# Dustin-Ray/capyCRYPT

Measured on NVIDIA B200. Metric: sha3_256_GBps, higher is better.
Workload: dtype u64

## Files before the change

### capycrypt_b200/csrc/sha3_api.cu

```cuda
#include <algorithm>
#include <cmath>
#include <cstdlib>
#include <memory>
#include <thread>
#include <type_traits>
#include <vector>

#include "internal.h"
#include "hostbatch.h"
#include "sponge.cuh"

namespace capy {

template <int LANES>
__global__ void __launch_bounds__(128)
    sha3_uniform_kernel(const uint8_t* __restrict__ data, uint64_t stride, uint64_t len, uint32_t suffix,
                        uint8_t* __restrict__ out, uint32_t out_bytes, uint64_t n) {
  const uint64_t i = (uint64_t)blockIdx.x * blockDim.x + threadIdx.x;
  if (i >= n) return;
  constexpr uint64_t RATE = 8ull * LANES;
  const uint2* q = reinterpret_cast<const uint2*>(data + i * stride);
  Lane a[25];
  state_zero(a);
  const uint64_t nfull = len / RATE;
  for (uint64_t b = 0; b < nfull; b++) {
#pragma unroll
    for (int j = 0; j < LANES; j++) {
      uint2 v = __ldg(q + j);
      a[j].lo ^= v.x;
      a[j].hi ^= v.y;
    }
    q += LANES;
    keccak_f1600(a);
  }
  const uint32_t rem = (uint32_t)(len - nfull * RATE);
#pragma unroll
  for (int j = 0; j < LANES; j++) {
    const uint32_t o = 8u * j;
    uint32_t lo = 0, hi = 0;
    if (o < rem) {
      uint2 v = __ldg(q + j);
      lo = v.x;
      hi = v.y;
      if (o + 8 > rem) {
        const uint32_t keep = rem - o;
        if (keep < 4) {
          lo &= (1u << (8 * keep)) - 1u;
          hi = 0;
        } else if (keep > 4) {
          hi &= (1u << (8 * (keep - 4))) - 1u;
        } else {
          hi = 0;
        }
      }
    }
    if (rem >= o && rem < o + 8) {
      const uint32_t k = rem - o;
      if (k < 4) lo |= suffix << (8 * k);
      else hi |= suffix << (8 * (k - 4));
    }
    a[j].lo ^= lo;
    a[j].hi ^= hi;
  }
  if (rem + 1 < RATE) a[LANES - 1].hi ^= 0x80000000u;
  keccak_f1600(a);

  uint8_t* o = out + i * (uint64_t)out_bytes;
  if ((out_bytes & 15u) == 0 && (reinterpret_cast<uintptr_t>(out) & 15u) == 0) {
#pragma unroll
    for (int j = 0; j < 4; j++)
      if (16u * j < out_bytes)
        reinterpret_cast<uint4*>(o)[j] = make_uint4(a[2 * j].lo, a[2 * j].hi, a[2 * j + 1].lo, a[2 * j + 1].hi);
  } else {
#pragma unroll
    for (int j = 0; j < 8; j++) {
      if (8u * j < out_bytes) reinterpret_cast<uint32_t*>(o)[2 * j] = a[j].lo;
      if (8u * j + 4 < out_bytes) reinterpret_cast<uint32_t*>(o)[2 * j + 1] = a[j].hi;
    }
  }
}

template <int LANES, int MSG_LANES>
__global__ void __launch_bounds__(128)
    sha3_short_kernel(const uint4* __restrict__ data, uint64_t stride16, uint32_t suffix, uint4* __restrict__ out,
                      uint32_t out_bytes, uint64_t n) {
  static_assert(MSG_LANES % 2 == 0 && MSG_LANES < LANES, "whole 16-byte loads, one block");
  const uint64_t i = (uint64_t)blockIdx.x * blockDim.x + threadIdx.x;
  if (i >= n) return;
  const uint4* q = data + i * stride16;
  Lane a[25];
  state_zero(a);
#pragma unroll
  for (int j = 0; j < MSG_LANES / 2; j++) {
    const uint4 v = __ldg(q + j);
    a[2 * j].lo = v.x;
    a[2 * j].hi = v.y;
    a[2 * j + 1].lo = v.z;
    a[2 * j + 1].hi = v.w;
  }
  a[MSG_LANES].lo = suffix;
  a[LANES - 1].hi ^= 0x80000000u;
  keccak_round(a, KECCAK_RC[0]);
#pragma unroll 1
  for (int r = 1; r < 23; r += 2) {
    keccak_round(a, KECCAK_RC[r]);
    keccak_round(a, KECCAK_RC[r + 1]);
  }
  keccak_round(a, KECCAK_RC[23]);
  uint4* o = out + i * (uint64_t)(out_bytes / 16);
#pragma unroll
  for (int j = 0; j < 4; j++)
    if (16u * j < out_bytes) o[j] = make_uint4(a[2 * j].lo, a[2 * j].hi, a[2 * j + 1].lo, a[2 * j + 1].hi);
}

template <int LANES>
__global__ void prefix_state_kernel(const uint8_t* prefix, uint32_t nblocks, uint64_t* state) {
  if (threadIdx.x != 0 || blockIdx.x != 0) return;
  Lane a[25];
  state_zero(a);
  for (uint32_t b = 0; b < nblocks; b++) {
    const uint8_t* p = prefix + (size_t)b * 8 * LANES;
#pragma unroll
    for (int j = 0; j < LANES; j++) {
      uint64_t v = 0;
      for (int k = 0; k < 8; k++) v |= (uint64_t)p[8 * j + k] << (8 * k);
      a[j].lo ^= (uint32_t)v;
      a[j].hi ^= (uint32_t)(v >> 32);
    }
    keccak_f1600(a);
  }
  for (int k = 0; k < 25; k++) state[k] = ((uint64_t)a[k].hi << 32) | a[k].lo;
}

constexpr uint32_t kLenBins = 1u << 14;
constexpr uint64_t kHostPlanMaxItems = 1ull << 18;

__device__ __forceinline__ uint32_t len_bin(const uint64_t* off, uint64_t i, uint32_t stride_bytes) {
  const uint64_t blocks = (off[i + 1] - off[i]) / stride_bytes;
  return blocks < kLenBins - 1 ? (uint32_t)blocks : kLenBins - 1;
}

__global__ void len_hist_kernel(const uint64_t* __restrict__ off, uint64_t n, uint32_t stride_bytes, uint32_t* hist) {
  const uint64_t i = (uint64_t)blockIdx.x * blockDim.x + threadIdx.x;
  if (i < n) atomicAdd(&hist[len_bin(off, i, stride_bytes)], 1u);
}

__global__ void __launch_bounds__(1024) len_scan_kernel(uint32_t* hist, uint32_t* summary) {
  __shared__ unsigned long long tot_s;
  __shared__ uint32_t max_s, bins_s;
  const uint32_t t = threadIdx.x;
  constexpr uint32_t PER = kLenBins / 1024;
  static_assert(PER == 16, "four uint4 per thread");
  if (t == 0) { tot_s = 0; max_s = 0; bins_s = 0; }
  __syncthreads();
  const uint32_t lo = kLenBins - (t + 1) * PER;
  uint32_t c[PER];
#pragma unroll
  for (int q = 0; q < 4; q++) {
    const uint4 v = reinterpret_cast<const uint4*>(hist + lo)[q];
    c[4 * q] = v.x; c[4 * q + 1] = v.y; c[4 * q + 2] = v.z; c[4 * q + 3] = v.w;
  }
  uint32_t sum = 0, nb = 0, mx = 0;
  unsigned long long tot = 0;
#pragma unroll
  for (int k = 0; k < (int)PER; k++) {
    sum += c[k];
    if (c[k]) { nb++; mx = lo + k; }
    tot += (unsigned long long)c[k] * (lo + k + 1);
  }
  if (sum) {
    atomicAdd(&tot_s, tot);
    atomicMax(&max_s, mx);
    atomicAdd(&bins_s, nb);
  }
  __syncthreads();
  uint32_t incl = sum;
#pragma unroll
  for (int d = 1; d < 32; d <<= 1) {
    const uint32_t v = __shfl_up_sync(0xffffffffu, incl, d);
    if ((t & 31) >= (uint32_t)d) incl += v;
  }
  __shared__ uint32_t wsum[32];
  if ((t & 31) == 31) wsum[t >> 5] = incl;
  __syncthreads();
  if (t < 32) {
    uint32_t w = wsum[t];
#pragma unroll
    for (int d = 1; d < 32; d <<= 1) {
      const uint32_t v = __shfl_up_sync(0xffffffffu, w, d);
      if (t >= (uint32_t)d) w += v;
    }
    wsum[t] = w;
  }
  __syncthreads();
  uint32_t run = incl - sum + ((t >> 5) ? wsum[(t >> 5) - 1] : 0u);
#pragma unroll
  for (int k = (int)PER - 1; k >= 0; k--) {
    const uint32_t cnt = c[k];
    c[k] = run;
    run += cnt;
  }
#pragma unroll
  for (int q = 0; q < 4; q++) reinterpret_cast<uint4*>(hist + lo)[q] = make_uint4(c[4 * q], c[4 * q + 1], c[4 * q + 2], c[4 * q + 3]);
  if (t == 0) {
    summary[0] = (uint32_t)tot_s;
    summary[1] = (uint32_t)(tot_s >> 32);
    summary[2] = max_s;
    summary[3] = bins_s;
  }
}

__global__ void len_scatter_kernel(const uint64_t* __restrict__ off, uint64_t n, uint32_t stride_bytes, uint32_t* cursor,
                                   uint32_t* __restrict__ order) {
  const uint64_t i = (uint64_t)blockIdx.x * blockDim.x + threadIdx.x;
  if (i < n) order[atomicAdd(&cursor[len_bin(off, i, stride_bytes)], 1u)] = (uint32_t)i;
}

constexpr double kPairChainRatio = 3.08 / 4.6;
constexpr int kMaxWarpCosched = 3;
constexpr double kWarpChainRatio[kMaxWarpCosched + 1] = {0.0, 2.06 / 4.6, 2.36 / 4.6, 3.00 / 4.6};

static void plan_tiers(const std::vector<uint32_t>& cum, uint64_t n, uint32_t max_blocks, double total_blocks, int sm_count,
                       uint64_t warp_items[kMaxWarpCosched], uint64_t* pair_items, int force_c = 0) {
  for (int c = 0; c < kMaxWarpCosched; c++) warp_items[c] = 0;
  *pair_items = 0;
  const size_t nb = cum.size();
  std::vector<double> work_above(nb);
  double acc = 0;
  for (size_t k = nb; k-- > 0;) {
    work_above[k] = acc;
    const uint64_t cnt = (k == 0 ? n : cum[k - 1]) - cum[k];
    acc += (double)cnt * (double)(k + 1);
  }
  auto longer_than = [&](double thr, uint64_t* count, double* work) {
    if (thr < 1.0) {
      *count = n;
      *work = total_blocks;
      return;
    }
    const size_t k = std::min<size_t>((size_t)thr - 1, nb - 1);
    *count = cum[k];
    *work = work_above[k];
  };
  const double l1 = (double)max_blocks;
  const int c_first = force_c >= 1 && force_c <= kMaxWarpCosched ? force_c : 1;
  for (double T = l1 * kWarpChainRatio[c_first]; T < l1; T *= 1.01) {
    uint64_t k_above[kMaxWarpCosched + 2];
    double w_above[kMaxWarpCosched + 2];
    k_above[0] = 0;
    w_above[0] = 0;
    for (int c = 1; c <= kMaxWarpCosched; c++) {
      const int next = c + 1;
      const double ratio = next <= kMaxWarpCosched ? kWarpChainRatio[next] : kPairChainRatio;
      longer_than(T / ratio, &k_above[c], &w_above[c]);
      if (force_c && c != force_c) {
        k_above[c] = c < force_c ? 0 : k_above[force_c];
        w_above[c] = c < force_c ? 0 : w_above[force_c];
      }
    }
    uint64_t k_fast;
    double w_fast;
    longer_than(T, &k_fast, &w_fast);
    if (k_above[kMaxWarpCosched] == 0 && T < l1 * kPairChainRatio) continue;
    uint64_t blocks = 0;
    double sm_time = 0;
    uint64_t cnt[kMaxWarpCosched];
    for (int c = 1; c <= kMaxWarpCosched; c++) {
      cnt[c - 1] = k_above[c] - k_above[c - 1];
      blocks += (cnt[c - 1] + 4 * c - 1) / (4 * c);
      sm_time += (w_above[c] - w_above[c - 1]) * kWarpChainRatio[c] / (4.0 * c);
    }
    const uint64_t k_p = k_fast - k_above[kMaxWarpCosched];
    blocks += (k_p + 63) / 64;
    sm_time += (w_fast - w_above[kMaxWarpCosched]) * kPairChainRatio / 64.0 + (total_blocks - w_fast) / 128.0;
    if (blocks + 1 > (uint64_t)sm_count) continue;
    if (sm_time > 0.95 * T * (double)sm_count) continue;
    if ((total_blocks - w_fast) / 128.0 > T * (double)((uint64_t)sm_count - blocks)) continue;
    for (int c = 0; c < kMaxWarpCosched; c++) warp_items[c] = cnt[c];
    *pair_items = k_p;
    return;
  }
}

template <int... Ls, class F>
static int with_lanes(int lanes, F&& f) {
  int rc = CAPY_ERR_BAD_ARG;
  (void)((lanes == Ls && ((rc = f(std::integral_constant<int, Ls>())), true)) || ...);
  return rc;
}

struct CudaFree {
  void operator()(void* p) const { cudaFree(p); }
};
template <class T>
using DevPtr = std::unique_ptr<T, CudaFree>;
template <class T>
static cudaError_t dev_alloc(DevPtr<T>& p, size_t bytes) {
  T* q = nullptr;
  const cudaError_t e = cudaMalloc(&q, bytes);
  if (e == cudaSuccess) p.reset(q);
  return e;
}

struct LenHist {
  uint64_t total_blocks = 0;
  uint32_t max_bin = 0;
  uint32_t bins = 0;
  std::vector<uint32_t> cnt;
};

static void host_len_hist(const uint64_t* h_off, uint64_t n, uint32_t stride_bytes, LenHist* h) {
  h->cnt.assign(kLenBins, 0);
  const double inv = 1.0 / (double)stride_bytes;
  for (uint64_t i = 0; i < n; i++) {
    const uint64_t len = h_off[i + 1] - h_off[i];
    uint64_t q = (uint64_t)((double)len * inv);
    if (q * stride_bytes > len) q--;
    else if ((q + 1) * stride_bytes <= len) q++;
    const uint32_t b = q < kLenBins - 1 ? (uint32_t)q : kLenBins - 1;
    if (h->cnt[b]++ == 0) h->bins++;
    if (b > h->max_bin) h->max_bin = b;
    h->total_blocks += (uint64_t)b + 1;
  }
}

static int device_len_hist(capy_ctx* ctx, cudaStream_t st, const uint64_t* d_off, uint64_t n, uint32_t stride_bytes,
                           uint32_t* hist, LenHist* h) {
  uint32_t* summary = hist + kLenBins;
  CAPY_CUDA(ctx, cudaMemsetAsync(hist, 0, (size_t)kLenBins * 4 + 64, st));
  len_hist_kernel<<<(unsigned)((n + 255) / 256), 256, 0, st>>>(d_off, n, stride_bytes, hist);
  len_scan_kernel<<<1, 1024, 0, st>>>(hist, summary);
  ctx->launches += 2;
  if (!h->cnt.empty()) return CAPY_OK;
  uint32_t h_sum[4];
  CAPY_CUDA(ctx, cudaMemcpyAsync(h_sum, summary, sizeof h_sum, cudaMemcpyDeviceToHost, st));
  CAPY_CUDA(ctx, cudaStreamSynchronize(st));
  h->total_blocks = (uint64_t)h_sum[0] | ((uint64_t)h_sum[1] << 32);
  h->max_bin = h_sum[2];
  h->bins = h_sum[3];
  return CAPY_OK;
}

static int plan_from_hist(capy_ctx* ctx, DeviceCtx& dc, cudaStream_t st, const uint64_t* d_off, uint64_t n,
                          uint32_t stride_bytes, const LenHist& h, uint32_t* hist, uint32_t* order, bool allow_pair,
                          int force_c, LaunchPlan* plan) {
  const uint32_t max_blocks = h.max_bin + 1;
  const double ideal = (double)h.total_blocks / (32.0 * 4.0 * dc.sm_count);
  if (allow_pair && max_blocks > 64 && (double)max_blocks > 1.05 * ideal) {
    std::vector<uint32_t> cum(kLenBins);
    if (!h.cnt.empty()) {
      uint32_t above = 0;
      for (uint32_t k = kLenBins; k-- > 0;) {
        cum[k] = above;
        above += h.cnt[k];
      }
    } else {
      CAPY_CUDA(ctx, cudaMemcpyAsync(cum.data(), hist, (size_t)kLenBins * 4, cudaMemcpyDeviceToHost, st));
      CAPY_CUDA(ctx, cudaStreamSynchronize(st));
    }
    plan_tiers(cum, n, max_blocks, (double)h.total_blocks, dc.sm_count, plan->warp_items, &plan->pair_items, force_c);
  }
  if (h.bins == 1) plan->uniform_blocks = max_blocks;
  if (h.bins > 1) {
    len_scatter_kernel<<<(unsigned)((n + 255) / 256), 256, 0, st>>>(d_off, n, stride_bytes, hist, order);
    ctx->launches++;
    CAPY_CUDA(ctx, cudaGetLastError());
    plan->order = order;
    plan->warps_per_smsp = 0;
    if ((double)max_blocks * 4.0 > 0.7 * ideal) {
      plan->warps_per_smsp = 3;
      if ((double)max_blocks * 3.0 > 0.7 * ideal) plan->warps_per_smsp = 2;
      if ((double)max_blocks * 2.0 > 0.7 * ideal) plan->warps_per_smsp = 1;
    }
  }
  return CAPY_OK;
}

static int plan_ragged(capy_ctx* ctx, DeviceCtx& dc, cudaStream_t st, const uint64_t* d_off, uint64_t n,
                       uint32_t stride_bytes, LaunchPlan* plan, bool allow_pair = true, int force_c = 0) {
  *plan = LaunchPlan();
  if (n < 1 || n > 0xffffffffull) return CAPY_OK;
  const uint64_t* h_off = host_off_find(dc, d_off, n);
  LenHist h;
  if (h_off) {
    const uint64_t len0 = h_off[1] - h_off[0];
    bool uniform = true;
    for (uint64_t i = 1; i < n && uniform; i++) uniform = (h_off[i + 1] - h_off[i]) == len0;
    if (uniform) {
      plan->uniform_blocks = len0 / stride_bytes + 1;
      return CAPY_OK;
    }
    if (n > kHostPlanMaxItems) h_off = nullptr;
    else host_len_hist(h_off, n, stride_bytes, &h);
  }
  const bool cached = ctx->plan_cache.load() != 0 && force_c == 0 && !h_off;
  if (cached) {
    for (PlanEntry& e : dc.plans)
      if (e.off == d_off && e.n == n && e.unit == stride_bytes && e.allow_pair == allow_pair) {
        e.last_use = ++dc.use_clock;
        *plan = e.plan;
        return CAPY_OK;
      }
  }
  uint32_t* hist = (uint32_t*)scratch_get(dc, st, kPlanHist, (size_t)kLenBins * 4 + 64);
  DevPtr<uint32_t> owned;
  if (cached && dev_alloc(owned, (size_t)n * 4) != cudaSuccess) {
    cudaGetLastError();
    return CAPY_ERR_OOM;
  }
  uint32_t* order = cached ? owned.get() : (uint32_t*)scratch_get(dc, st, kPlanOrder, (size_t)n * 4);
  if (!hist || !order) return CAPY_ERR_OOM;
  int rc = device_len_hist(ctx, st, d_off, n, stride_bytes, hist, &h);
  if (rc) return rc;
  rc = plan_from_hist(ctx, dc, st, d_off, n, stride_bytes, h, hist, order, allow_pair, force_c, plan);
  if (rc) return rc;
  if (cached) {
    if (!plan->order) owned.reset();
    if (dc.plans.size() >= kMaxPlanEntries) {
      size_t lru = 0;
      for (size_t k = 1; k < dc.plans.size(); k++)
        if (dc.plans[k].last_use < dc.plans[lru].last_use) lru = k;
      if (dc.plans[lru].owned_order) cudaFree(dc.plans[lru].owned_order);
      dc.plans.erase(dc.plans.begin() + lru);
    }
    PlanEntry e;
    e.off = d_off;
    e.n = n;
    e.unit = stride_bytes;
    e.allow_pair = allow_pair;
    e.plan = *plan;
    e.owned_order = owned.release();
    e.last_use = ++dc.use_clock;
    dc.plans.push_back(e);
  }
  return CAPY_OK;
}

template <class Kernel>
static cudaError_t throttle(Kernel* kernel, const LaunchPlan& plan, unsigned* block, size_t* smem) {
  *smem = 0;
  if (plan.warps_per_smsp < 1 || plan.warps_per_smsp > 3) return cudaSuccess;
  *block = 128;
  *smem = (size_t)(227 * 1024 / plan.warps_per_smsp) - 1024;
  return cudaFuncSetAttribute(kernel, cudaFuncAttributeMaxDynamicSharedMemorySize, 226 * 1024);
}

template <int LANES>
static int launch_sponge_t(capy_ctx* ctx, cudaStream_t stream, SpongeJob J, unsigned block, const LaunchPlan& plan) {
  if (plan.tiered()) {
    const uint64_t warp_items = plan.warp_items[0] + plan.warp_items[1] + plan.warp_items[2], pair_items = plan.pair_items;
    SpongeTiers tiers;
    uint32_t warp_blocks = 0;
    uint64_t rank = 0;
    for (int c = 0; c < 3; c++) {
      tiers.first_block[c] = warp_blocks;
      tiers.first_rank[c] = rank;
      warp_blocks += grid_for(plan.warp_items[c], 4 * (c + 1));
      rank += plan.warp_items[c];
    }
    tiers.warp_blocks = warp_blocks;
    tiers.pair_blocks = grid_for(2 * pair_items, 128);
    const unsigned solo_blocks = grid_for(J.n - pair_items - warp_items, 128);
    J.warp_items = warp_items;
    J.first = warp_items + pair_items;
    CAPY_CUDA(ctx, cudaFuncSetAttribute(sponge_tiered_kernel<LANES>, cudaFuncAttributeMaxDynamicSharedMemorySize, 226 * 1024));
    sponge_tiered_kernel<LANES><<<warp_blocks + tiers.pair_blocks + solo_blocks, 384, 226 * 1024, stream>>>(J, tiers);
    ctx->launches++;
    CAPY_CUDA(ctx, cudaGetLastError());
    return CAPY_OK;
  }
  size_t smem;
  CAPY_CUDA(ctx, throttle(sponge_kernel<LANES>, plan, &block, &smem));
  sponge_kernel<LANES><<<grid_for(J.n, block), block, smem, stream>>>(J);
  ctx->launches++;
  CAPY_CUDA(ctx, cudaGetLastError());
  return CAPY_OK;
}

static unsigned pick_block(uint64_t n, int sm_count, int threads_per_sm) {
  unsigned best = 128;
  double best_eff = -1.0;
  for (unsigned bs : {128u, 64u, 32u}) {
    const uint64_t blocks = (n + bs - 1) / bs;
    const uint64_t slots = (uint64_t)sm_count * (threads_per_sm / bs);
    const uint64_t waves = (blocks + slots - 1) / slots;
    const double per_sm = (double)blocks / sm_count;
    const double busiest = waves > 1 ? (double)waves * (threads_per_sm / bs) : (double)((blocks + sm_count - 1) / sm_count);
    const double eff = per_sm / busiest;
    if (eff > best_eff + 0.02) {
      best_eff = eff;
      best = bs;
    }
  }
  return best;
}

static int job_lanes(const SpongeJob& J) { return (int)(J.rate / 8); }

static int launch_sponge(capy_ctx* ctx, DeviceCtx& dc, cudaStream_t stream, const SpongeJob& J, const LaunchPlan& plan) {
  if (J.n == 0) return CAPY_OK;
  const unsigned block = pick_block(J.n, dc.sm_count, 384);
  return with_lanes<9, 13, 17, 18, 19, 21>(job_lanes(J), [&](auto L) {
    return launch_sponge_t<decltype(L)::value>(ctx, stream, J, block, plan);
  });
}

static int launch_sponge_seq(capy_ctx* ctx, DeviceCtx& dc, cudaStream_t stream, const SpongeJob& A, const SpongeJob& B,
                             const LaunchPlan& plan) {
  const int rc = launch_sponge(ctx, dc, stream, A, plan);
  if (rc) return rc;
  return launch_sponge(ctx, dc, stream, B, plan);
}

static bool chain_jobs_fit(int sm_count, uint64_t n) {
  if (getenv("CAPY_NO_CHAIN_SPLIT") || sm_count < 1) return false;
  return (n + 127) / 128 >= (uint64_t)CAPY_SPONGE_MINB * (uint64_t)sm_count;
}

static bool chain_cut(int sm_count, uint64_t n, uint64_t absorb_blocks, uint64_t squeeze_extra, uint64_t* cut) {
  if (!chain_jobs_fit(sm_count, n)) return false;
  const uint64_t warps = (n + 31) / 32, sched = 4ull * (uint64_t)sm_count;
  if (warps > 8 * sched) return false;
  auto fill = [&](uint64_t w) {
    const double x = (double)w / (double)sched;
    return x / std::ceil(x);
  };
  if (fill(2 * warps) < fill(warps) + 0.04) return false;
  const uint64_t perms = absorb_blocks + squeeze_extra;
  if (perms < 12) return false;
  uint64_t k = (perms + 1) / 2;
  if (k > absorb_blocks) k = absorb_blocks;
  if (3 * k < perms) return false;
  *cut = k;
  return true;
}

static int launch_chain_jobs(capy_ctx* ctx, DeviceCtx& dc, cudaStream_t stream, const SpongeJob& J0, const SpongeJob& J1,
                             bool data_dependent) {
  const uint32_t nb = (uint32_t)((J0.n + 127) / 128);
  uint32_t* sync = (uint32_t*)scratch_get(dc, stream, kChainSync, ((size_t)nb + 1) * sizeof(uint32_t));
  if (!sync) return CAPY_ERR_OOM;
  CAPY_CUDA(ctx, cudaMemsetAsync(sync, 0, ((size_t)nb + 1) * sizeof(uint32_t), stream));
  SpongeChain C;
  C.j[0] = J0;
  C.j[1] = J1;
  C.sync = sync;
  C.blocks_per_job = nb;
  C.data_dependent = data_dependent ? 1u : 0u;
  return with_lanes<9, 13, 17, 18, 19, 21>(job_lanes(J0), [&](auto L) {
    sponge_chain_kernel<decltype(L)::value><<<2 * nb, 128, 0, stream>>>(C);
    ctx->launches++;
    CAPY_CUDA(ctx, cudaGetLastError());
    return CAPY_OK;
  });
}

static int launch_sponge_chain(capy_ctx* ctx, DeviceCtx& dc, cudaStream_t stream, const SpongeJob& J, uint64_t cut) {
  uint64_t* states = (uint64_t*)scratch_get(dc, stream, kChainStates, (size_t)J.n * 25 * sizeof(uint64_t));
  if (!states) return CAPY_ERR_OOM;
  SpongeJob J0 = J, J1 = J;
  J0.chain_out = states;
  J0.stop_block = J.skip_blocks + cut;
  J1.chain_in = states;
  J1.skip_blocks = (uint32_t)(J.skip_blocks + cut);
  return launch_chain_jobs(ctx, dc, stream, J0, J1, false);
}

static bool uniform_cut(const DeviceCtx& dc, const SpongeJob& J, const LaunchPlan& plan, uint64_t* cut) {
  if (J.out_off || J.xor_in || plan.order || (J.rate & 7u) != 0) return false;
  const uint64_t msg_blocks = J.off ? plan.uniform_blocks : J.msg_len / J.rate + 1;
  if (!msg_blocks) return false;
  uint64_t absorb = msg_blocks;
  if (J.keys) absorb += ((uint64_t)J.key_len + 8) / J.w + 1;
  if (!J.skip_blocks) absorb += J.prefix_len / J.rate;
  const uint64_t sq = 8ull * J.sq_lanes, squeeze_extra = J.out_bytes ? (J.out_bytes + sq - 1) / sq - 1 : 0;
  return chain_cut(dc.sm_count, J.n, absorb, squeeze_extra, cut);
}

static int run_sponge(capy_ctx* ctx, DeviceCtx& dc, cudaStream_t stream, SpongeJob J, const LaunchPlan& plan) {
  J.order = plan.order;
  uint64_t cut;
  if (uniform_cut(dc, J, plan, &cut)) return launch_sponge_chain(ctx, dc, stream, J, cut);
  return launch_sponge(ctx, dc, stream, J, plan);
}

static int launch_sha3(capy_ctx* ctx, DeviceCtx& dc, cudaStream_t stream, int d, const uint8_t* data, const uint64_t* off,
                       uint64_t msg_len, uint64_t stride, uint64_t n, uint8_t* out, uint32_t flags = 0,
                       bool tail_readable = true) {
  if (!valid_secparam(d)) return CAPY_ERR_BAD_SECPARAM;
  if (n == 0) return CAPY_OK;
  if (!off && !tail_readable && (msg_len & 7u) != 0 && n > 1 && (reinterpret_cast<uintptr_t>(data) & 7u) == 0 &&
      (stride & 7u) == 0 && (reinterpret_cast<uintptr_t>(out) & 3u) == 0) {
    int rc = launch_sha3(ctx, dc, stream, d, data, nullptr, msg_len, stride, n - 1, out, flags, true);
    if (rc) return rc;
    return launch_sha3(ctx, dc, stream, d, data + (n - 1) * stride, nullptr, msg_len, stride, 1, out + (n - 1) * (uint64_t)(d / 8),
                       flags, false);
  }
  const uint32_t rate = (1600 - sha3_capacity(d)) / 8;
  const int lanes = (int)rate / 8;
  if (!off && (reinterpret_cast<uintptr_t>(data) & 15u) == 0 && (reinterpret_cast<uintptr_t>(out) & 15u) == 0 &&
      (stride & 15u) == 0 && (d == 256 || d == 512) && msg_len >= 16 && (msg_len & 15u) == 0 && msg_len < rate) {
    const unsigned block = 128, grid = grid_for(n, block);
    const uint4* dq = reinterpret_cast<const uint4*>(data);
    uint4* oq = reinterpret_cast<uint4*>(out);
    const uint64_t s16 = stride / 16;
    const int msg_lanes = (int)(msg_len / 8);
    const int rc = d == 256 ? with_lanes<2, 4, 6, 8, 10, 12, 14, 16>(msg_lanes, [&](auto M) {
      sha3_short_kernel<17, decltype(M)::value><<<grid, block, 0, stream>>>(dq, s16, 0x06u, oq, 32, n);
      return CAPY_OK;
    }) : with_lanes<2, 4, 6, 8>(msg_lanes, [&](auto M) {
      sha3_short_kernel<9, decltype(M)::value><<<grid, block, 0, stream>>>(dq, s16, 0x06u, oq, 64, n);
      return CAPY_OK;
    });
    if (rc) return rc;
    ctx->launches++;
    CAPY_CUDA(ctx, cudaGetLastError());
    return CAPY_OK;
  }
  SpongeJob J{};
  J.data = data;
  J.off = off;
  J.msg_len = msg_len;
  J.msg_stride = stride;
  J.trailer_len = 1;
  J.sha3_suffix = 1;
  J.rate = rate;
  J.out = out;
  J.out_stride = J.out_bytes = (uint64_t)d / 8;
  J.sq_lanes = (1600 - d) / 64;
  J.n = n;
  uint64_t cut;
  if (!off && !uniform_cut(dc, J, LaunchPlan(), &cut) && (reinterpret_cast<uintptr_t>(data) & 7u) == 0 &&
      (stride & 7u) == 0 && (reinterpret_cast<uintptr_t>(out) & 3u) == 0 && (tail_readable || (msg_len & 7u) == 0)) {
    const uint32_t suffix = (msg_len % 136u == 135u) ? 0x86u : 0x06u;
    const unsigned block = 128, grid = grid_for(n, block);
    return with_lanes<9, 13, 17, 18>(lanes, [&](auto L) {
      sha3_uniform_kernel<decltype(L)::value><<<grid, block, 0, stream>>>(data, stride, msg_len, suffix, out, d / 8, n);
      ctx->launches++;
      CAPY_CUDA(ctx, cudaGetLastError());
      return CAPY_OK;
    });
  }
  LaunchPlan plan;
  if (off && !(flags & CAPY_FLAG_NO_SORT)) {
    int rc = plan_ragged(ctx, dc, stream, off, n, rate, &plan, !(flags & CAPY_FLAG_NO_PAIR),
                         (int)((flags >> CAPY_FLAG_WARP_COSCHED_SHIFT) & 3u));
    if (rc) return rc;
  }
  return run_sponge(ctx, dc, stream, J, plan);
}

static void host_left_encode(std::string& o, uint64_t v) {
  if (v == 0) {
    o.push_back(1);
    o.push_back(0);
    return;
  }
  int nb = 8;
  while (nb > 1 && ((v >> (8 * (nb - 1))) & 0xFF) == 0) nb--;
  o.push_back((char)nb);
  for (int i = nb - 1; i >= 0; i--) o.push_back((char)((v >> (8 * i)) & 0xFF));
}
static void host_encode_string(std::string& o, const uint8_t* s, size_t n) {
  host_left_encode(o, (uint64_t)n * 8);
  o.append(reinterpret_cast<const char*>(s), n);
}

static int get_prefix(capy_ctx* ctx, DeviceCtx& dc, cudaStream_t stream, int d, const uint8_t* fn, uint32_t fn_len,
                      const uint8_t* cs, uint32_t cs_len, PrefixState** out) {
  std::string key;
  key.push_back((char)(d >> 8));
  key.push_back((char)d);
  host_left_encode(key, fn_len);
  key.append(reinterpret_cast<const char*>(fn), fn_len);
  key.append(reinterpret_cast<const char*>(cs), cs_len);
  auto it = dc.prefix_cache.find(key);
  if (it != dc.prefix_cache.end()) {
    it->second.last_use = ++dc.use_clock;
    *out = &it->second;
    return CAPY_OK;
  }
  if (dc.prefix_cache.size() >= kMaxPrefixEntries) {
    auto lru = dc.prefix_cache.begin();
    for (auto k = dc.prefix_cache.begin(); k != dc.prefix_cache.end(); ++k)
      if (k->second.last_use < lru->second.last_use) lru = k;
    if (lru->second.d_state) cudaFree(lru->second.d_state);
    if (lru->second.d_prefix) cudaFree(lru->second.d_prefix);
    dc.prefix_cache.erase(lru);
  }
  const uint32_t w = bytepad_value(d);
  std::string p;
  host_left_encode(p, w);
  host_encode_string(p, fn, fn_len);
  host_encode_string(p, cs, cs_len);
  p.append(w - p.size() % w, '\0');
  PrefixState ps;
  ps.prefix_len = (uint32_t)p.size();
  DevPtr<uint8_t> d_prefix;
  DevPtr<uint64_t> d_state;
  CAPY_CUDA(ctx, dev_alloc(d_prefix, p.size()));
  CAPY_CUDA(ctx, dev_alloc(d_state, 25 * sizeof(uint64_t)));
  CAPY_CUDA(ctx, cudaMemcpyAsync(d_prefix.get(), p.data(), p.size(), cudaMemcpyHostToDevice, stream));
  if (w % 8 == 0) {
    ps.skip_blocks = ps.prefix_len / w;
    const int rc = with_lanes<17, 19, 21>((int)(w / 8), [&](auto L) {
      prefix_state_kernel<decltype(L)::value><<<1, 32, 0, stream>>>(d_prefix.get(), ps.skip_blocks, d_state.get());
      ctx->launches++;
      CAPY_CUDA(ctx, cudaGetLastError());
      return CAPY_OK;
    });
    if (rc) return rc;
  } else {
    ps.skip_blocks = 0;
  }
  CAPY_CUDA(ctx, cudaStreamSynchronize(stream));
  ps.d_prefix = d_prefix.release();
  ps.d_state = d_state.release();
  ps.last_use = ++dc.use_clock;
  auto ins = dc.prefix_cache.emplace(key, ps);
  *out = &ins.first->second;
  return CAPY_OK;
}

static void fill_cshake_common(SpongeJob& J, int d, const PrefixState* ps) {
  const uint32_t w = bytepad_value(d);
  J.prefix = ps->d_prefix;
  J.prefix_len = ps->prefix_len;
  J.init_state = ps->skip_blocks ? ps->d_state : nullptr;
  J.skip_blocks = ps->skip_blocks;
  J.w = w;
  J.rate = (1600 - d) / 8;
  J.sq_lanes = (1600 - d) / 64;
}

static int launch_cshake(capy_ctx* ctx, DeviceCtx& dc, cudaStream_t stream, int d, const uint8_t* data,
                         const uint64_t* off, uint64_t n, const uint8_t* fn, uint32_t fn_len, const uint8_t* cs,
                         uint32_t cs_len, uint64_t out_bits, uint8_t* out) {
  if (!valid_secparam(d)) return CAPY_ERR_BAD_SECPARAM;
  if (n == 0 || out_bits / 8 == 0) return CAPY_OK;
  PrefixState* ps;
  int rc = get_prefix(ctx, dc, stream, d, fn, fn_len, cs, cs_len, &ps);
  if (rc) return rc;
  SpongeJob J{};
  fill_cshake_common(J, d, ps);
  J.data = data;
  J.off = off;
  J.trailer = 0x04;
  J.trailer_len = 1;
  if (fn_len == 0 && cs_len == 0) J.q4_rate = (1600 - sha3_capacity(d)) / 8;
  J.out = out;
  J.out_stride = J.out_bytes = out_bits / 8;
  J.n = n;
  LaunchPlan plan;
  rc = plan_ragged(ctx, dc, stream, off, n, J.rate & ~7u, &plan);
  if (rc) return rc;
  return run_sponge(ctx, dc, stream, J, plan);
}

static int build_kmac_job(capy_ctx* ctx, DeviceCtx& dc, cudaStream_t stream, const KmacDevArgs& a, SpongeJob* out) {
  static const uint8_t kKmac[4] = {'K', 'M', 'A', 'C'};
  PrefixState* ps;
  int rc = get_prefix(ctx, dc, stream, a.d_bits, kKmac, 4, a.custom, a.custom_len, &ps);
  if (rc) return rc;
  SpongeJob J{};
  fill_cshake_common(J, a.d_bits, ps);
  J.keys = a.keys;
  J.key_off = a.key_off;
  J.key_len = (uint32_t)a.key_len;
  J.key_stride = a.key_stride;
  J.data = a.data;
  J.off = a.off;
  J.msg_len = a.msg_len;
  J.msg_stride = a.msg_stride;
  J.trailer = 0x040100u;
  J.trailer_len = 3;
  J.out = a.out;
  J.out_off = a.out_off;
  J.out_stride = a.out_stride;
  J.out_bytes = a.out_bytes;
  J.xor_in = a.xor_in;
  J.n = a.n;
  *out = J;
  return CAPY_OK;
}

static int plan_kmac(capy_ctx* ctx, DeviceCtx& dc, cudaStream_t stream, const KmacDevArgs& a, const SpongeJob& J, LaunchPlan* plan) {
  *plan = LaunchPlan();
  if (a.no_sort) return CAPY_OK;
  if (a.off) return plan_ragged(ctx, dc, stream, a.off, a.n, J.rate & ~7u, plan);
  if (a.out_off) return plan_ragged(ctx, dc, stream, a.out_off, a.n, 8u * J.sq_lanes, plan);
  return CAPY_OK;
}

int launch_kmac_xof(capy_ctx* ctx, DeviceCtx& dc, cudaStream_t stream, const KmacDevArgs& a) {
  if (!valid_secparam(a.d_bits)) return CAPY_ERR_BAD_SECPARAM;
  if (a.n == 0) return CAPY_OK;
  if (!a.out_off && a.out_bytes == 0) return CAPY_OK;
  SpongeJob J;
  int rc = build_kmac_job(ctx, dc, stream, a, &J);
  if (rc) return rc;
  LaunchPlan plan;
  rc = plan_kmac(ctx, dc, stream, a, J, &plan);
  if (rc) return rc;
  return run_sponge(ctx, dc, stream, J, plan);
}

template <int LANES>
static int launch_sponge2_t(capy_ctx* ctx, cudaStream_t stream, const SpongeJob& A, const SpongeJob& B, unsigned block,
                            const LaunchPlan& plan) {
  SpongeJob2 JJ;
  JJ.j[0] = A;
  JJ.j[1] = B;
  size_t smem;
  CAPY_CUDA(ctx, throttle(sponge_kernel2<LANES>, plan, &block, &smem));
  const uint64_t warps = 2 * ((A.n + 31) / 32);
  sponge_kernel2<LANES><<<grid_for(warps * 32, block), block, smem, stream>>>(JJ);
  ctx->launches++;
  CAPY_CUDA(ctx, cudaGetLastError());
  return CAPY_OK;
}

int launch_kmac_xof2(capy_ctx* ctx, DeviceCtx& dc, cudaStream_t stream, const KmacDevArgs& a, const KmacDevArgs& b) {
  if (!valid_secparam(a.d_bits) || a.d_bits != b.d_bits || a.n != b.n) return CAPY_ERR_BAD_ARG;
  if (a.n == 0) return CAPY_OK;
  SpongeJob JA, JB;
  int rc = build_kmac_job(ctx, dc, stream, a, &JA);
  if (rc) return rc;
  rc = build_kmac_job(ctx, dc, stream, b, &JB);
  if (rc) return rc;
  LaunchPlan plan;
  rc = plan_kmac(ctx, dc, stream, a, JA, &plan);
  if (rc) return rc;
  JA.order = JB.order = plan.order;
  if (plan.tiered()) return launch_sponge_seq(ctx, dc, stream, JA, JB, plan);
  const unsigned block = pick_block(2 * a.n, dc.sm_count, 384);
  return with_lanes<17, 19, 21>(job_lanes(JA), [&](auto L) {
    return launch_sponge2_t<decltype(L)::value>(ctx, stream, JA, JB, block, plan);
  });
}

int launch_kmac_xof_dep(capy_ctx* ctx, DeviceCtx& dc, cudaStream_t stream, const KmacDevArgs& first, const KmacDevArgs& second) {
  if (!valid_secparam(first.d_bits) || first.d_bits != second.d_bits || first.n != second.n) return CAPY_ERR_BAD_ARG;
  if (first.n == 0) return CAPY_OK;
  SpongeJob J0, J1;
  int rc = build_kmac_job(ctx, dc, stream, first, &J0);
  if (rc) return rc;
  rc = build_kmac_job(ctx, dc, stream, second, &J1);
  if (rc) return rc;
  LaunchPlan plan;
  rc = plan_kmac(ctx, dc, stream, second, J1, &plan);
  if (rc) return rc;
  J0.order = J1.order = plan.order;
  if (plan.tiered() || (J0.rate & 7u) != 0 || !chain_jobs_fit(dc.sm_count, first.n))
    return launch_sponge_seq(ctx, dc, stream, J0, J1, plan);
  return launch_chain_jobs(ctx, dc, stream, J0, J1, true);
}

}

using namespace capy;

extern "C" {

int capy_plan_tiers(const uint32_t* items_longer_than, uint32_t n_bins, uint64_t n, uint32_t max_blocks, uint64_t total_blocks,
                    int sm_count, uint64_t* warp_items, uint64_t* pair_items) {
  uint64_t w[3];
  int rc = capy_plan_tiers3(items_longer_than, n_bins, n, max_blocks, total_blocks, sm_count, w, pair_items);
  if (rc == CAPY_OK && warp_items) *warp_items = w[0] + w[1] + w[2];
  return warp_items ? rc : CAPY_ERR_BAD_ARG;
}

int capy_plan_tiers3(const uint32_t* items_longer_than, uint32_t n_bins, uint64_t n, uint32_t max_blocks, uint64_t total_blocks,
                     int sm_count, uint64_t* warp_items_by_sharing, uint64_t* pair_items) {
  if (!items_longer_than || !n_bins || !warp_items_by_sharing || !pair_items || sm_count < 2) return CAPY_ERR_BAD_ARG;
  std::vector<uint32_t> cum(items_longer_than, items_longer_than + n_bins);
  plan_tiers(cum, n, max_blocks, (double)total_blocks, sm_count, warp_items_by_sharing, pair_items);
  return CAPY_OK;
}

int capy_chain_cut(int sm_count, uint64_t n, uint64_t absorb_blocks, uint64_t squeeze_extra, uint64_t* cut_after_blocks) {
  if (!cut_after_blocks) return CAPY_ERR_BAD_ARG;
  *cut_after_blocks = 0;
  return chain_cut(sm_count, n, absorb_blocks, squeeze_extra, cut_after_blocks) ? 1 : 0;
}

int capy_lpt_shares(const uint64_t* off, uint64_t n, uint32_t parts, uint32_t unit_bytes, uint64_t per_item_cost,
                    uint32_t* owner) {
  if (!off || !owner || parts == 0 || unit_bytes == 0) return CAPY_ERR_BAD_ARG;
  auto shares = lpt_shares(off, n, parts, unit_bytes, per_item_cost);
  for (size_t d = 0; d < shares.size(); d++)
    for (const Run& r : shares[d].runs)
      for (uint64_t i = r.i0; i < r.i1; i++) owner[i] = (uint32_t)d;
  return CAPY_OK;
}

int capy_sha3_batch_dev(capy_ctx* ctx, int dev_index, void* stream, int d_bits, const uint8_t* d_data,
                        const uint64_t* d_off, uint64_t n, uint8_t* d_digests, uint32_t flags) {
  if (n && (!d_data || !d_off || !d_digests)) return CAPY_ERR_BAD_ARG;
  CAPY_DEV_PROLOGUE
  return launch_sha3(ctx, dc, st, d_bits, d_data, d_off, 0, 0, n, d_digests, flags);
}

int capy_sha3_batch_fixed_dev(capy_ctx* ctx, int dev_index, void* stream, int d_bits, const uint8_t* d_data,
                              uint64_t msg_len, uint64_t stride, uint64_t n, uint8_t* d_digests, uint32_t) {
  if ((n && (!d_data || !d_digests)) || stride < msg_len) return CAPY_ERR_BAD_ARG;
  CAPY_DEV_PROLOGUE
  return launch_sha3(ctx, dc, st, d_bits, d_data, nullptr, msg_len, stride, n, d_digests, 0, false);
}

int capy_sha3_batch(capy_ctx* ctx, int d_bits, const uint8_t* data, const uint64_t* off, uint64_t n, uint8_t* digests,
                    uint32_t flags) {
  if (!ctx || (n && (!data || !off || !digests))) return CAPY_ERR_BAD_ARG;
  if (!valid_secparam(d_bits)) return CAPY_ERR_BAD_SECPARAM;
  if (n == 0) return CAPY_OK;
  const size_t ob = (size_t)d_bits / 8;
  if (ctx->devs.size() > 1) {
    const uint32_t rate = (1600 - sha3_capacity(d_bits)) / 8;
    auto shares = lpt_shares(off, n, ctx->devs.size(), rate, 2);
    bool scattered = false;
    for (const DeviceShare& s : shares) scattered |= s.runs.size() > 1;
    if (scattered) {
      std::vector<Range> slots;
      for (size_t k = 0; k < shares.size(); k++) slots.push_back({k, k + 1});
      return for_each_device(ctx, slots, [&](DeviceCtx& dc, Range slot, int*) -> int {
        const DeviceShare& sh = shares[slot.i0];
        if (sh.items == 0) return CAPY_OK;
        cudaStream_t st = dc.streams[0];
        uint8_t* d_data = (uint8_t*)scratch_get(dc, st, kHost0, (size_t)sh.bytes + 16);
        uint64_t* d_off = (uint64_t*)scratch_get(dc, st, kHost1, (size_t)(sh.items + 1) * 8);
        uint8_t* d_out = (uint8_t*)scratch_get(dc, st, kHost2, (size_t)sh.items * ob);
        if (!d_data || !d_off || !d_out) return CAPY_ERR_OOM;
        std::vector<uint64_t> loc(sh.items + 1);
        uint64_t at = 0, j = 0;
        for (const Run& r : sh.runs) {
          const uint64_t b0 = off[r.i0], b1 = off[r.i1];
          if (b1 > b0) {
            const int rc = copy_in(ctx, dc, st, kHost0, d_data + at, data + b0, (size_t)(b1 - b0));
            if (rc) return rc;
          }
          for (uint64_t i = r.i0; i < r.i1; i++) loc[j++] = at + (off[i] - b0);
          at += b1 - b0;
        }
        loc[j] = at;
        CAPY_CUDA(ctx, cudaMemcpyAsync(d_off, loc.data(), (size_t)(sh.items + 1) * 8, cudaMemcpyHostToDevice, st));
        host_off_register(dc, d_off, loc.data(), sh.items + 1);
        int rc = launch_sha3(ctx, dc, st, d_bits, d_data, d_off, 0, 0, sh.items, d_out, flags);
        if (rc) return rc;
        j = 0;
        for (const Run& r : sh.runs) {
          rc = copy_out(ctx, dc, st, kHost2, digests + r.i0 * ob, d_out + j * ob, (size_t)(r.i1 - r.i0) * ob);
          if (rc) return rc;
          j += r.i1 - r.i0;
        }
        CAPY_CUDA(ctx, cudaStreamSynchronize(st));
        return CAPY_OK;
      });
    }
  }
  auto shards = split_items(off, 0, 0, n, ctx->devs.size(), 200);
  return for_each_device(ctx, shards, [&](DeviceCtx& dc, Range sh, int*) -> int {
    auto chunks = split_items(off, 0, sh.i0, sh.i1, ragged_chunk_count(off, sh.i0, sh.i1, 0), 200);
    return run_chunks(ctx, dc, chunks, nullptr, [&](cudaStream_t st, Range ch, int*) -> int {
      StagedPacked sp;
      int rc = stage_packed(ctx, dc, st, kHost0, kHost1, data, off, ch.i0, ch.i1, &sp);
      if (rc) return rc;
      uint8_t* d_out = (uint8_t*)scratch_get(dc, st, kHost2, (size_t)(ch.i1 - ch.i0) * ob);
      if (!d_out) return CAPY_ERR_OOM;
      rc = launch_sha3(ctx, dc, st, d_bits, sp.d_base, sp.d_off, 0, 0, ch.i1 - ch.i0, d_out, flags);
      if (rc) return rc;
      return copy_out(ctx, dc, st, kHost2, digests + ch.i0 * ob, d_out, (size_t)(ch.i1 - ch.i0) * ob);
    });
  });
}

int capy_sha3_batch_fixed(capy_ctx* ctx, int d_bits, const uint8_t* data, uint64_t msg_len, uint64_t stride, uint64_t n,
                          uint8_t* digests, uint32_t) {
  if (!ctx || (n && (!data || !digests)) || stride < msg_len) return CAPY_ERR_BAD_ARG;
  if (!valid_secparam(d_bits)) return CAPY_ERR_BAD_SECPARAM;
  if (n == 0) return CAPY_OK;
  const size_t ob = (size_t)d_bits / 8;
  auto shards = split_items(nullptr, stride, 0, n, ctx->devs.size(), 0);
  return for_each_device(ctx, shards, [&](DeviceCtx& dc, Range sh, int*) -> int {
    auto chunks = split_items(nullptr, stride, sh.i0, sh.i1, chunk_count((sh.i1 - sh.i0) * stride, sh.i1 - sh.i0), 0);
    return run_chunks(ctx, dc, chunks, nullptr, [&](cudaStream_t st, Range ch, int*) -> int {
      const uint64_t cnt = ch.i1 - ch.i0;
      const size_t in_bytes = (size_t)((cnt - 1) * stride + msg_len);
      uint8_t* d_in = (uint8_t*)scratch_get(dc, st, kHost0, in_bytes + 16);
      uint8_t* d_out = (uint8_t*)scratch_get(dc, st, kHost2, (size_t)cnt * ob);
      if (!d_in || !d_out) return CAPY_ERR_OOM;
      int rc = copy_in(ctx, dc, st, kHost0, d_in, data + ch.i0 * stride, in_bytes);
      if (rc) return rc;
      rc = launch_sha3(ctx, dc, st, d_bits, d_in, nullptr, msg_len, stride, cnt, d_out);
      if (rc) return rc;
      return copy_out(ctx, dc, st, kHost2, digests + ch.i0 * ob, d_out, (size_t)cnt * ob);
    });
  });
}

int capy_cshake_batch_dev(capy_ctx* ctx, int dev_index, void* stream, int d_bits, const uint8_t* d_data,
                          const uint64_t* d_off, uint64_t n, const uint8_t* fn_name, uint32_t fn_len,
                          const uint8_t* custom, uint32_t custom_len, uint64_t out_bits, uint8_t* d_out) {
  if ((n && (!d_data || !d_off || !d_out)) || (fn_len && !fn_name) || (custom_len && !custom)) return CAPY_ERR_BAD_ARG;
  CAPY_DEV_PROLOGUE
  return launch_cshake(ctx, dc, st, d_bits, d_data, d_off, n, fn_name, fn_len, custom, custom_len, out_bits, d_out);
}

int capy_cshake_batch(capy_ctx* ctx, int d_bits, const uint8_t* data, const uint64_t* off, uint64_t n,
                      const uint8_t* fn_name, uint32_t fn_len, const uint8_t* custom, uint32_t custom_len,
                      uint64_t out_bits, uint8_t* out) {
  if (!ctx || (n && (!data || !off || !out)) || (fn_len && !fn_name) || (custom_len && !custom)) return CAPY_ERR_BAD_ARG;
  if (!valid_secparam(d_bits)) return CAPY_ERR_BAD_SECPARAM;
  const size_t ob = (size_t)(out_bits / 8);
  if (n == 0 || ob == 0) return CAPY_OK;
  auto shards = split_items(off, 0, 0, n, ctx->devs.size(), 200 + ob);
  return for_each_device(ctx, shards, [&](DeviceCtx& dc, Range sh, int*) -> int {
    auto chunks = split_items(off, 0, sh.i0, sh.i1,
                              ragged_chunk_count(off, sh.i0, sh.i1, (sh.i1 - sh.i0) * ob), 200 + ob);
    return run_chunks(ctx, dc, chunks, nullptr, [&](cudaStream_t st, Range ch, int*) -> int {
      StagedPacked sp;
      int rc = stage_packed(ctx, dc, st, kHost0, kHost1, data, off, ch.i0, ch.i1, &sp);
      if (rc) return rc;
      uint8_t* d_out = (uint8_t*)scratch_get(dc, st, kHost2, (size_t)(ch.i1 - ch.i0) * ob);
      if (!d_out) return CAPY_ERR_OOM;
      rc = launch_cshake(ctx, dc, st, d_bits, sp.d_base, sp.d_off, ch.i1 - ch.i0, fn_name, fn_len, custom, custom_len,
                         out_bits, d_out);
      if (rc) return rc;
      return copy_out(ctx, dc, st, kHost2, out + ch.i0 * ob, d_out, (size_t)(ch.i1 - ch.i0) * ob);
    });
  });
}

int capy_kmac_xof_batch_dev(capy_ctx* ctx, int dev_index, void* stream, int d_bits, const uint8_t* d_keys,
                            const uint64_t* d_key_off, const uint8_t* d_data, const uint64_t* d_off, uint64_t n,
                            const uint8_t* custom, uint32_t custom_len, uint64_t out_bits, const uint64_t* d_out_off,
                            uint8_t* d_out) {
  if ((n && (!d_keys || !d_key_off || !d_data || !d_off || !d_out)) || (custom_len && !custom)) return CAPY_ERR_BAD_ARG;
  CAPY_DEV_PROLOGUE
  KmacDevArgs a{};
  a.d_bits = d_bits;
  a.keys = d_keys;
  a.key_off = d_key_off;
  a.data = d_data;
  a.off = d_off;
  a.n = n;
  a.custom = custom;
  a.custom_len = custom_len;
  a.out_bytes = a.out_stride = out_bits / 8;
  a.out_off = d_out_off;
  a.out = d_out;
  return launch_kmac_xof(ctx, dc, st, a);
}

int capy_kmac_xof_batch_fixed_dev(capy_ctx* ctx, int dev_index, void* stream, int d_bits, const uint8_t* d_keys,
                                  uint64_t key_len, uint64_t key_stride, const uint8_t* d_data, uint64_t msg_len,
                                  uint64_t msg_stride, uint64_t n, const uint8_t* custom, uint32_t custom_len,
                                  uint64_t out_bits, uint8_t* d_out) {
  if ((n && (!d_keys || !d_out)) || (n && msg_len && !d_data) || (custom_len && !custom) || key_stride < key_len ||
      msg_stride < msg_len)
    return CAPY_ERR_BAD_ARG;
  CAPY_DEV_PROLOGUE
  KmacDevArgs a{};
  a.d_bits = d_bits;
  a.keys = d_keys;
  a.key_len = key_len;
  a.key_stride = key_stride;
  a.data = d_data ? d_data : d_keys;
  a.msg_len = msg_len;
  a.msg_stride = msg_stride;
  a.n = n;
  a.custom = custom;
  a.custom_len = custom_len;
  a.out_bytes = a.out_stride = out_bits / 8;
  a.out = d_out;
  return launch_kmac_xof(ctx, dc, st, a);
}

int capy_kmac_xof_batch(capy_ctx* ctx, int d_bits, const uint8_t* keys, const uint64_t* key_off, const uint8_t* data,
                        const uint64_t* off, uint64_t n, const uint8_t* custom, uint32_t custom_len, uint64_t out_bits,
                        const uint64_t* out_off, uint8_t* out) {
  if (!ctx || (n && (!keys || !key_off || !data || !off || !out)) || (custom_len && !custom)) return CAPY_ERR_BAD_ARG;
  if (!valid_secparam(d_bits)) return CAPY_ERR_BAD_SECPARAM;
  const size_t ob = (size_t)(out_bits / 8);
  if (n == 0 || (!out_off && ob == 0)) return CAPY_OK;
  auto out_begin = [&](uint64_t i) -> uint64_t { return out_off ? out_off[i] : i * ob; };
  auto shards = split_items(off, 0, 0, n, ctx->devs.size(), 400 + ob);
  return for_each_device(ctx, shards, [&](DeviceCtx& dc, Range sh, int*) -> int {
    const uint64_t tot = off[sh.i1] - off[sh.i0] + (out_begin(sh.i1) - out_begin(sh.i0));
    auto chunks = split_items(off, 0, sh.i0, sh.i1, ragged_chunk_count(off, sh.i0, sh.i1, tot - (off[sh.i1] - off[sh.i0])), 400 + ob);
    return run_chunks(ctx, dc, chunks, nullptr, [&](cudaStream_t st, Range ch, int*) -> int {
      const uint64_t cnt = ch.i1 - ch.i0;
      StagedPacked sx, sk;
      int rc = stage_packed(ctx, dc, st, kHost0, kHost1, data, off, ch.i0, ch.i1, &sx);
      if (rc) return rc;
      rc = stage_packed(ctx, dc, st, kHost2, kHost3, keys, key_off, ch.i0, ch.i1, &sk);
      if (rc) return rc;
      const uint64_t ob0 = out_begin(ch.i0), ob1 = out_begin(ch.i1);
      uint8_t* d_out = (uint8_t*)scratch_get(dc, st, kHost4, (size_t)(ob1 - ob0) + 16);
      if (!d_out) return CAPY_ERR_OOM;
      const uint64_t* d_out_off = nullptr;
      uint8_t* d_out_base = d_out;
      if (out_off) {
        uint64_t* p = (uint64_t*)scratch_get(dc, st, kHost5, (size_t)(cnt + 1) * 8);
        if (!p) return CAPY_ERR_OOM;
        CAPY_CUDA(ctx, cudaMemcpyAsync(p, out_off + ch.i0, (size_t)(cnt + 1) * 8, cudaMemcpyHostToDevice, st));
        d_out_off = p;
        d_out_base = reinterpret_cast<uint8_t*>(reinterpret_cast<uintptr_t>(d_out) - (uintptr_t)ob0);
      }
      KmacDevArgs a{};
      a.d_bits = d_bits;
      a.keys = sk.d_base;
      a.key_off = sk.d_off;
      a.data = sx.d_base;
      a.off = sx.d_off;
      a.n = cnt;
      a.custom = custom;
      a.custom_len = custom_len;
      a.out_bytes = a.out_stride = ob;
      a.out_off = d_out_off;
      a.out = d_out_base;
      rc = launch_kmac_xof(ctx, dc, st, a);
      if (rc) return rc;
      if (ob1 > ob0) return copy_out(ctx, dc, st, kHost4, out + ob0, d_out, (size_t)(ob1 - ob0));
      return CAPY_OK;
    });
  });
}

int capy_fips_shake_batch_dev(capy_ctx* ctx, int dev_index, void* stream, int shake_bits, const uint8_t* d_data,
                              const uint64_t* d_off, uint64_t n, uint64_t out_bytes, uint8_t* d_out) {
  if (!dev_index_ok(ctx, dev_index) || (n && (!d_data || !d_off || !d_out)) || (shake_bits != 128 && shake_bits != 256))
    return CAPY_ERR_BAD_ARG;
  if (n == 0 || out_bytes == 0) return CAPY_OK;
  CAPY_DEV_PROLOGUE
  SpongeJob J{};
  J.data = d_data;
  J.off = d_off;
  J.trailer = 0x1F;
  J.trailer_len = 1;
  J.fips_pad = 1;
  J.rate = (1600 - 2 * shake_bits) / 8;
  J.sq_lanes = J.rate / 8;
  J.out = d_out;
  J.out_stride = J.out_bytes = out_bytes;
  J.n = n;
  LaunchPlan plan;
  int rc = plan_ragged(ctx, dc, st, d_off, n, J.rate, &plan);
  if (rc) return rc;
  return run_sponge(ctx, dc, st, J, plan);
}

}
```

Measured before the change: 270.9.

## Bitslice short-message Keccak across warp lanes using shuffle-based rotations

Rewrites the short-message SHA3 kernel to compute 32 messages per warp in bitsliced form. Each lane holds two bit positions of every state lane, so the rho rotations become warp shuffles and the round constant becomes a predicated bit flip. Message words are transposed with a shuffle/funnel-shift network on input and transposed back on output. Launch bounds are also raised to request 4 blocks per SM. The cost is a large number of shuffle instructions, which run at lower throughput than funnel shifts, plus extra transpose work. The output path now assumes the digest size equals the capacity-derived lane count.

```diff
diff --git a/capycrypt_b200/csrc/keccak_bs.cuh b/capycrypt_b200/csrc/keccak_bs.cuh
--- /dev/null
+++ b/capycrypt_b200/csrc/keccak_bs.cuh
@@ -0,0 +1,116 @@
+#pragma once
+#include <cstdint>
+
+#include "keccak.cuh"
+
+namespace capy {
+
+static __device__ const uint2 KECCAK_RC_BITS[32] = {
+    {0x50F4F1u, 0x0DB916u}, {0x000000u, 0x8C7F94u}, {0x000000u, 0x000000u}, {0x000000u, 0x327356u},
+    {0x000000u, 0x000000u}, {0x000000u, 0x000000u}, {0x000000u, 0x000000u}, {0x000000u, 0xB5D4DEu},
+    {0x000000u, 0x000000u}, {0x000000u, 0x000000u}, {0x000000u, 0x000000u}, {0x000000u, 0x000000u},
+    {0x000000u, 0x000000u}, {0x000000u, 0x000000u}, {0x000000u, 0x000000u}, {0x000000u, 0xD81C68u},
+    {0x000000u, 0x000000u}, {0x000000u, 0x000000u}, {0x000000u, 0x000000u}, {0x000000u, 0x000000u},
+    {0x000000u, 0x000000u}, {0x000000u, 0x000000u}, {0x000000u, 0x000000u}, {0x000000u, 0x000000u},
+    {0x000000u, 0x000000u}, {0x000000u, 0x000000u}, {0x000000u, 0x000000u}, {0x000000u, 0x000000u},
+    {0x000000u, 0x000000u}, {0x000000u, 0x000000u}, {0x000000u, 0x000000u}, {0x000000u, 0xBBE0CCu}};
+
+template <int K>
+__device__ __forceinline__ uint32_t bs_from(uint32_t v, uint32_t lane) {
+  if constexpr (K % 32 == 0) return v;
+  else return __shfl_sync(0xffffffffu, v, (int)(lane - (uint32_t)K));
+}
+
+template <int R>
+__device__ __forceinline__ void bs_rot(uint32_t (&b)[2], uint32_t t0, uint32_t t1, uint32_t lane) {
+  if constexpr (R % 2 == 0) {
+    b[0] = bs_from<R / 2>(t0, lane);
+    b[1] = bs_from<R / 2>(t1, lane);
+  } else {
+    b[0] = bs_from<(R + 1) / 2>(t1, lane);
+    b[1] = bs_from<(R - 1) / 2>(t0, lane);
+  }
+}
+
+#define CAPY_BS_RHO_PI(X, Y, R)                                                                       \
+  bs_rot<(R)>(b[(Y) + 5 * ((2 * (X) + 3 * (Y)) % 5)],                                                 \
+              lop_xor3(a[(X) + 5 * (Y)][0], c[((X) + 4) % 5][0], n[((X) + 1) % 5][0]),                \
+              lop_xor3(a[(X) + 5 * (Y)][1], c[((X) + 4) % 5][1], n[((X) + 1) % 5][1]), lane);
+
+__device__ __forceinline__ uint32_t bs_flip_if(uint32_t v, uint32_t rounds, uint32_t round) {
+  asm("{\n\t.reg .pred p;\n\t.reg .b32 t;\n\tand.b32 t, %1, %2;\n\tsetp.ne.u32 p, t, 0;\n\t@p not.b32 %0, %0;\n\t}"
+      : "+r"(v)
+      : "r"(rounds), "r"(round));
+  return v;
+}
+
+__device__ __forceinline__ void keccak_bs_round(uint32_t (&a)[25][2], uint32_t lane, uint2 rc, uint32_t round) {
+  uint32_t c[5][2], n[5][2], b[25][2];
+#pragma unroll
+  for (int x = 0; x < 5; x++) {
+#pragma unroll
+    for (int h = 0; h < 2; h++) c[x][h] = lop_xor3(lop_xor3(a[x][h], a[x + 5][h], a[x + 10][h]), a[x + 15][h], a[x + 20][h]);
+    n[x][0] = bs_from<1>(c[x][1], lane);
+    n[x][1] = c[x][0];
+  }
+  CAPY_BS_RHO_PI(0, 0, 0)  CAPY_BS_RHO_PI(1, 0, 1)  CAPY_BS_RHO_PI(2, 0, 62) CAPY_BS_RHO_PI(3, 0, 28) CAPY_BS_RHO_PI(4, 0, 27)
+  CAPY_BS_RHO_PI(0, 1, 36) CAPY_BS_RHO_PI(1, 1, 44) CAPY_BS_RHO_PI(2, 1, 6)  CAPY_BS_RHO_PI(3, 1, 55) CAPY_BS_RHO_PI(4, 1, 20)
+  CAPY_BS_RHO_PI(0, 2, 3)  CAPY_BS_RHO_PI(1, 2, 10) CAPY_BS_RHO_PI(2, 2, 43) CAPY_BS_RHO_PI(3, 2, 25) CAPY_BS_RHO_PI(4, 2, 39)
+  CAPY_BS_RHO_PI(0, 3, 41) CAPY_BS_RHO_PI(1, 3, 45) CAPY_BS_RHO_PI(2, 3, 15) CAPY_BS_RHO_PI(3, 3, 21) CAPY_BS_RHO_PI(4, 3, 8)
+  CAPY_BS_RHO_PI(0, 4, 18) CAPY_BS_RHO_PI(1, 4, 2)  CAPY_BS_RHO_PI(2, 4, 61) CAPY_BS_RHO_PI(3, 4, 56) CAPY_BS_RHO_PI(4, 4, 14)
+#pragma unroll
+  for (int y = 0; y < 5; y++) {
+#pragma unroll
+    for (int x = 0; x < 5; x++) {
+#pragma unroll
+      for (int h = 0; h < 2; h++)
+        a[x + 5 * y][h] = lop_chi(b[x + 5 * y][h], b[(x + 1) % 5 + 5 * y][h], b[(x + 2) % 5 + 5 * y][h]);
+    }
+  }
+  a[0][0] = bs_flip_if(a[0][0], rc.x, round);
+  a[0][1] = bs_flip_if(a[0][1], rc.y, round);
+}
+#undef CAPY_BS_RHO_PI
+
+struct BsTranspose {
+  uint32_t rot[5], keep[5];
+  __device__ __forceinline__ explicit BsTranspose(uint32_t lane) {
+#pragma unroll
+    for (int k = 0; k < 5; k++) {
+      const uint32_t d = 16u >> k;
+      const uint32_t lo_bits = k == 0 ? 0x0000FFFFu : k == 1 ? 0x00FF00FFu : k == 2 ? 0x0F0F0F0Fu : k == 3 ? 0x33333333u : 0x55555555u;
+      const bool upper = lane & d;
+      rot[k] = upper ? 32u - d : d;
+      keep[k] = upper ? ~lo_bits : lo_bits;
+    }
+  }
+  __device__ __forceinline__ uint32_t operator()(uint32_t x) const {
+#pragma unroll
+    for (int k = 0; k < 5; k++) {
+      const uint32_t y = __shfl_xor_sync(0xffffffffu, x, 16u >> k);
+      const uint32_t r = __funnelshift_l(y, y, rot[k]);
+      asm("lop3.b32 %0, %0, %1, %2, 0xE4;" : "+r"(x) : "r"(r), "r"(keep[k]));
+    }
+    return x;
+  }
+};
+
+__device__ __forceinline__ void bs_gather(uint32_t (&w)[2], uint32_t lo, uint32_t hi, uint32_t lane) {
+#pragma unroll
+  for (int h = 0; h < 2; h++) {
+    const int src = (int)(2 * lane + h);
+    const uint32_t l = __shfl_sync(0xffffffffu, lo, src);
+    const uint32_t u = __shfl_sync(0xffffffffu, hi, src);
+    w[h] = lane < 16 ? l : u;
+  }
+}
+
+__device__ __forceinline__ void bs_scatter(uint32_t& lo, uint32_t& hi, const uint32_t (&w)[2], uint32_t lane) {
+  const int src = (int)(lane >> 1);
+  const uint32_t l0 = __shfl_sync(0xffffffffu, w[0], src), l1 = __shfl_sync(0xffffffffu, w[1], src);
+  const uint32_t u0 = __shfl_sync(0xffffffffu, w[0], src + 16), u1 = __shfl_sync(0xffffffffu, w[1], src + 16);
+  lo = lane & 1 ? l1 : l0;
+  hi = lane & 1 ? u1 : u0;
+}
+
+}
diff --git a/capycrypt_b200/csrc/sha3_api.cu b/capycrypt_b200/csrc/sha3_api.cu
--- a/capycrypt_b200/csrc/sha3_api.cu
+++ b/capycrypt_b200/csrc/sha3_api.cu
@@ -8,6 +8,7 @@
 
 #include "internal.h"
 #include "hostbatch.h"
+#include "keccak_bs.cuh"
 #include "sponge.cuh"
 
 namespace capy {
@@ -81,36 +82,59 @@
 }
 
 template <int LANES, int MSG_LANES>
-__global__ void __launch_bounds__(128)
+__global__ void __launch_bounds__(128, 4)
     sha3_short_kernel(const uint4* __restrict__ data, uint64_t stride16, uint32_t suffix, uint4* __restrict__ out,
                       uint32_t out_bytes, uint64_t n) {
   static_assert(MSG_LANES % 2 == 0 && MSG_LANES < LANES, "whole 16-byte loads, one block");
+  constexpr int OUT_LANES = (200 - 8 * LANES) / 16;
+  const uint32_t lane = threadIdx.x & 31u;
   const uint64_t i = (uint64_t)blockIdx.x * blockDim.x + threadIdx.x;
-  if (i >= n) return;
-  const uint4* q = data + i * stride16;
-  Lane a[25];
-  state_zero(a);
-#pragma unroll
-  for (int j = 0; j < MSG_LANES / 2; j++) {
-    const uint4 v = __ldg(q + j);
-    a[2 * j].lo = v.x;
-    a[2 * j].hi = v.y;
-    a[2 * j + 1].lo = v.z;
-    a[2 * j + 1].hi = v.w;
-  }
-  a[MSG_LANES].lo = suffix;
-  a[LANES - 1].hi ^= 0x80000000u;
-  keccak_round(a, KECCAK_RC[0]);
+  if (i - lane >= n) return;
+  const bool live = i < n;
+  const BsTranspose transpose(lane);
+
+  uint32_t a[25][2];
+  {
+    const uint4* q = data + i * stride16;
+    uint32_t w[2 * MSG_LANES];
+#pragma unroll
+    for (int j = 0; j < MSG_LANES / 2; j++) {
+      const uint4 v = live ? __ldg(q + j) : make_uint4(0u, 0u, 0u, 0u);
+      w[4 * j] = v.x;
+      w[4 * j + 1] = v.y;
+      w[4 * j + 2] = v.z;
+      w[4 * j + 3] = v.w;
+    }
+#pragma unroll
+    for (int j = 0; j < 2 * MSG_LANES; j++) w[j] = transpose(w[j]);
+#pragma unroll
+    for (int l = 0; l < MSG_LANES; l++) bs_gather(a[l], w[2 * l], w[2 * l + 1], lane);
+  }
+#pragma unroll
+  for (int l = MSG_LANES; l < 25; l++) a[l][0] = a[l][1] = 0u;
+  const uint32_t pad = (uint32_t)((uint64_t)suffix >> (2 * lane));
+  a[MSG_LANES][0] = 0u - (pad & 1u);
+  a[MSG_LANES][1] = 0u - ((pad >> 1) & 1u);
+  a[LANES - 1][1] ^= lane == 31 ? 0xFFFFFFFFu : 0u;
+
+  const uint2 rc = __ldg(&KECCAK_RC_BITS[lane]);
+  keccak_bs_round(a, lane, rc, 1u);
 #pragma unroll 1
   for (int r = 1; r < 23; r += 2) {
-    keccak_round(a, KECCAK_RC[r]);
-    keccak_round(a, KECCAK_RC[r + 1]);
-  }
-  keccak_round(a, KECCAK_RC[23]);
+    keccak_bs_round(a, lane, rc, 1u << r);
+    keccak_bs_round(a, lane, rc, 2u << r);
+  }
+  keccak_bs_round(a, lane, rc, 1u << 23);
+
+  uint32_t w[2 * OUT_LANES];
+#pragma unroll
+  for (int l = 0; l < OUT_LANES; l++) bs_scatter(w[2 * l], w[2 * l + 1], a[l], lane);
+#pragma unroll
+  for (int j = 0; j < 2 * OUT_LANES; j++) w[j] = transpose(w[j]);
+  if (!live) return;
   uint4* o = out + i * (uint64_t)(out_bytes / 16);
 #pragma unroll
-  for (int j = 0; j < 4; j++)
-    if (16u * j < out_bytes) o[j] = make_uint4(a[2 * j].lo, a[2 * j].hi, a[2 * j + 1].lo, a[2 * j + 1].hi);
+  for (int j = 0; j < OUT_LANES / 2; j++) o[j] = make_uint4(w[4 * j], w[4 * j + 1], w[4 * j + 2], w[4 * j + 3]);
 }
 
 template <int LANES>
```

Result: faster. 309.6 (median of 6 runs) (+14.3%).
